# 0xWOLAND/halo2-prover

Hardware: AMD Instinct MI355X
Metric: MSM+NTT field-ops/s (higher is better)
Workload: dtype u32 limbs (256-bit modular)

## Files before the change

### halo2_prover_amd/csrc/h2_curve29.hpp

```cpp
#pragma once
#include "h2_curve.hpp"
#include "h2_field29.hpp"

namespace h2 {

constexpr int XYZZ29_WORDS = 36;

template <class CV>
struct Affine29 {
  using F = Fe29<typename CV::Base>;
  F x, y;
  H2_HD bool is_identity() const { return x.is_zero_exact() && y.is_zero_exact(); }
};

template <class CV>
struct Xyzz29 {
  using F = Fe29<typename CV::Base>;
  F x, y, zz, zzz;
  H2_HD bool is_identity() const { return zz.is_zero_exact(); }
  static H2_HD Xyzz29 identity() { return Xyzz29{F::zero(), F::zero(), F::zero(), F::zero()}; }
};

template <class CV>
H2_HD Affine29<CV> affine29_load(const void* p, bool negate) {
  using B = typename CV::Base;
  const char* c = reinterpret_cast<const char*>(p);
  Affine29<CV> a{fe29_unpack(fe_load<B>(c)), fe29_unpack(fe_load<B>(c + 32))};
  if (negate) a.y = fe29_neg(a.y);
  return a;
}
template <class CV>
H2_HD void affine29_store_table(void* p, const Affine<CV>& a) {
  using B = typename CV::Base;
  char* c = reinterpret_cast<char*>(p);
  if (a.is_identity()) {
    fe_store<B>(c, Fe<B>::zero());
    fe_store<B>(c + 32, Fe<B>::zero());
    return;
  }
  fe_store<B>(c, fe29_pack(fe29_from_api(a.x)));
  fe_store<B>(c + 32, fe29_pack(fe29_from_api(a.y)));
}

template <class CV>
H2_HD Xyzz29<CV> xyzz29_load(const uint32_t* p) {
  Xyzz29<CV> r;
#pragma unroll
  for (int i = 0; i < 9; i++) {
    r.x.v[i] = (int32_t)p[i];
    r.y.v[i] = (int32_t)p[9 + i];
    r.zz.v[i] = (int32_t)p[18 + i];
    r.zzz.v[i] = (int32_t)p[27 + i];
  }
  return r;
}
template <class CV>
H2_HD void xyzz29_store(uint32_t* p, const Xyzz29<CV>& a) {
#pragma unroll
  for (int i = 0; i < 9; i++) {
    p[i] = (uint32_t)a.x.v[i];
    p[9 + i] = (uint32_t)a.y.v[i];
    p[18 + i] = (uint32_t)a.zz.v[i];
    p[27 + i] = (uint32_t)a.zzz.v[i];
  }
}

template <class CV>
H2_HD Fe29<typename CV::Base> fe29_one() {
  using B = typename CV::Base;
  return fe29_from_api(Fe<B>::one());
}

template <class CV>
H2_HD Xyzz29<CV> xyzz29_from_affine(const Affine29<CV>& a) {
  if (a.is_identity()) return Xyzz29<CV>::identity();
  const Fe29<typename CV::Base> one = fe29_one<CV>();
  return Xyzz29<CV>{a.x, fe29_norm(a.y), one, one};
}

template <class CV>
H2_HD Xyzz29<CV> xyzz29_double_affine(const Affine29<CV>& a) {
  using F = Fe29<typename CV::Base>;
  if (a.is_identity() || fe29_is_zero_mod_p(a.y)) return Xyzz29<CV>::identity();
  const F u = fe29_norm(fe29_add(a.y, a.y));
  const F v = fe29_sqr(u);
  const F w = fe29_mul(u, v);
  const F s = fe29_mul(a.x, v);
  const F xx = fe29_sqr(a.x);
  const F m = fe29_norm(fe29_add(fe29_add(xx, xx), xx));
  const F x3 = fe29_norm(fe29_sub(fe29_sub(fe29_sqr(m), s), s));
  const F y3 = fe29_mul_sub(m, fe29_sub(s, x3), w, a.y);
  return Xyzz29<CV>{x3, y3, v, w};
}

template <class CV>
H2_HD Xyzz29<CV> xyzz29_double(const Xyzz29<CV>& p) {
  using F = Fe29<typename CV::Base>;
  if (p.is_identity() || fe29_is_zero_mod_p(p.y)) return Xyzz29<CV>::identity();
  const F u = fe29_norm(fe29_add(p.y, p.y));
  const F v = fe29_sqr(u);
  const F w = fe29_mul(u, v);
  const F s = fe29_mul(p.x, v);
  const F xx = fe29_sqr(p.x);
  const F m = fe29_norm(fe29_add(fe29_add(xx, xx), xx));
  const F x3 = fe29_norm(fe29_sub(fe29_sub(fe29_sqr(m), s), s));
  const F y3 = fe29_mul_sub(m, fe29_sub(s, x3), w, p.y);
  return Xyzz29<CV>{x3, y3, fe29_mul(v, p.zz), fe29_mul(w, p.zzz)};
}

template <class CV>
H2_HD Xyzz29<CV> xyzz29_add_affine(const Xyzz29<CV>& acc, const Affine29<CV>& q) {
  using F = Fe29<typename CV::Base>;
  if (q.is_identity()) return acc;
  if (acc.is_identity()) return xyzz29_from_affine(q);
  const F u2 = fe29_mul(q.x, acc.zz);
  const F s2 = fe29_mul(q.y, acc.zzz);
  const F p = fe29_sub(u2, acc.x);
  const F r = fe29_sub(s2, acc.y);
  if (fe29_is_zero_mod_p(p)) {
    if (fe29_is_zero_mod_p(r)) return xyzz29_double_affine(q);
    return Xyzz29<CV>::identity();
  }
  const F pp = fe29_sqr(p);
  const F ppp = fe29_mul(p, pp);
  const F qq = fe29_mul(acc.x, pp);
  const F x3 = fe29_norm(fe29_sub(fe29_sub(fe29_sub(fe29_sqr(r), ppp), qq), qq));
  const F y3 = fe29_mul_sub(r, fe29_sub(qq, x3), acc.y, ppp);
  return Xyzz29<CV>{x3, y3, fe29_mul(acc.zz, pp), fe29_mul(acc.zzz, ppp)};
}

template <class CV>
H2_HD Xyzz29<CV> xyzz29_add(const Xyzz29<CV>& a, const Xyzz29<CV>& b) {
  using F = Fe29<typename CV::Base>;
  if (a.is_identity()) return b;
  if (b.is_identity()) return a;
  const F u1 = fe29_mul(a.x, b.zz);
  const F u2 = fe29_mul(b.x, a.zz);
  const F s1 = fe29_mul(a.y, b.zzz);
  const F s2 = fe29_mul(b.y, a.zzz);
  const F p = fe29_sub(u2, u1);
  const F r = fe29_sub(s2, s1);
  if (fe29_is_zero_mod_p(p)) {
    if (fe29_is_zero_mod_p(r)) return xyzz29_double(a);
    return Xyzz29<CV>::identity();
  }
  const F pp = fe29_sqr(p);
  const F ppp = fe29_mul(p, pp);
  const F qq = fe29_mul(u1, pp);
  const F x3 = fe29_norm(fe29_sub(fe29_sub(fe29_sub(fe29_sqr(r), ppp), qq), qq));
  const F y3 = fe29_mul_sub(r, fe29_sub(qq, x3), s1, ppp);
  return Xyzz29<CV>{x3, y3, fe29_mul(fe29_mul(a.zz, b.zz), pp), fe29_mul(fe29_mul(a.zzz, b.zzz), ppp)};
}

template <class CV>
H2_HD Xyzz<CV> xyzz29_to_api(const Xyzz29<CV>& p) {
  if (p.is_identity()) return Xyzz<CV>::identity();
  return Xyzz<CV>{fe29_to_api(p.x), fe29_to_api(p.y), fe29_to_api(p.zz), fe29_to_api(p.zzz)};
}

}
```

### halo2_prover_amd/csrc/h2_field29.hpp

```cpp
#pragma once
#include "h2_field.hpp"

namespace h2 {

constexpr uint32_t L29_MASK = (1u << 29) - 1;

template <class FP>
struct Fe29 {
  int32_t v[9];
  static H2_HD Fe29 zero() {
    Fe29 r;
#pragma unroll
    for (int i = 0; i < 9; i++) r.v[i] = 0;
    return r;
  }
  H2_HD bool is_zero_exact() const {
    int32_t o = 0;
#pragma unroll
    for (int i = 0; i < 9; i++) o |= v[i];
    return o == 0;
  }
};

template <class FP>
H2_HD constexpr uint32_t fe29_p(int j) {
  const int bit = 29 * j;
  const int w = bit / 32, s = bit % 32;
  const uint64_t lo = w < 8 ? FP::P(w) : 0, hi = w + 1 < 8 ? FP::P(w + 1) : 0;
  return (uint32_t)(((lo | (hi << 32)) >> s) & L29_MASK);
}

template <class FP>
H2_HD Fe29<FP> fe29_unpack(const Fe<FP>& a) {
  Fe29<FP> r;
#pragma unroll
  for (int j = 0; j < 9; j++) {
    const int bit = 29 * j, w = bit >> 5, s = bit & 31;
    const uint64_t lo = a.v[w], hi = w + 1 < 8 ? a.v[w + 1] : 0;
    r.v[j] = (int32_t)((uint32_t)((lo | (hi << 32)) >> s) & L29_MASK);
  }
  return r;
}
template <class FP>
H2_HD Fe<FP> fe29_pack(const Fe29<FP>& a) {
  Fe<FP> r;
#pragma unroll
  for (int w = 0; w < 8; w++) {
    const int bit = 32 * w, j = bit / 29, off = bit % 29;
    uint64_t x = (uint64_t)(uint32_t)a.v[j] >> off;
    x |= (uint64_t)(uint32_t)a.v[j + 1] << (29 - off);
    if (j + 2 < 9) x |= (uint64_t)(uint32_t)a.v[j + 2] << (58 - off);
    r.v[w] = (uint32_t)x;
  }
  return r;
}

template <class FP>
H2_HD Fe29<FP> fe29_add(const Fe29<FP>& a, const Fe29<FP>& b) {
  Fe29<FP> r;
#pragma unroll
  for (int i = 0; i < 9; i++) r.v[i] = a.v[i] + b.v[i];
  return r;
}
template <class FP>
H2_HD Fe29<FP> fe29_sub(const Fe29<FP>& a, const Fe29<FP>& b) {
  Fe29<FP> r;
#pragma unroll
  for (int i = 0; i < 9; i++) r.v[i] = a.v[i] - b.v[i];
  return r;
}
template <class FP>
H2_HD Fe29<FP> fe29_neg(const Fe29<FP>& a) {
  Fe29<FP> r;
#pragma unroll
  for (int i = 0; i < 9; i++) r.v[i] = -a.v[i];
  return r;
}
template <class FP>
H2_HD Fe29<FP> fe29_norm(const Fe29<FP>& a) {
  Fe29<FP> r;
  int32_t carry = 0;
#pragma unroll
  for (int i = 0; i < 8; i++) {
    const int32_t x = a.v[i] + carry;
    r.v[i] = (int32_t)((uint32_t)x & L29_MASK);
    carry = x >> 29;
  }
  r.v[8] = a.v[8] + carry;
  return r;
}

H2_HD int32_t fe29_opaque(int32_t x) {
#if defined(__HIP_DEVICE_COMPILE__)
  asm("" : "+v"(x));
#endif
  return x;
}
namespace detail29 {
H2_HD int32_t fe29_hidden(int32_t c) {
#if defined(__HIP_DEVICE_COMPILE__)
  asm("" : "+s"(c));
#endif
  return c;
}
template <class FP, int J, bool UP>
H2_HD void msub_p(int64_t& acc, int32_t m) {
  constexpr uint32_t pj = fe29_p<FP>(J);
  if constexpr (UP) {
    if constexpr (pj == 0) {
    } else if constexpr (pj == 1) {
      acc += m;
    } else if constexpr ((pj & (pj - 1)) == 0) {
      acc += (int64_t)m << __builtin_ctz(pj);
    } else {
      acc += (int64_t)m * (int32_t)pj;
    }
  } else if constexpr (pj == 0) {
  } else if constexpr (__builtin_popcount(pj) <= 2) {
    acc += (int64_t)m * fe29_hidden(-(int32_t)pj);
  } else {
    acc += (int64_t)m * -(int32_t)pj;
  }
}
template <class FP, bool UP>
H2_HD int32_t mont_step(int64_t& acc) {
  constexpr uint32_t pinv = (0u - (FP::INV & L29_MASK)) & L29_MASK;
  if constexpr (UP) {
    constexpr uint32_t ninv = FP::INV & L29_MASK;
    const int32_t m = ninv == L29_MASK ? (int32_t)((0u - (uint32_t)acc) & L29_MASK)
                                       : (int32_t)(((uint32_t)acc * ninv) & L29_MASK);
    msub_p<FP, 0, true>(acc, m);
    return m;
  } else if constexpr (pinv == 1) {
    return fe29_opaque((int32_t)((uint32_t)acc & L29_MASK));
  } else {
    const int32_t m = fe29_opaque((int32_t)(((uint32_t)acc * pinv) & L29_MASK));
    msub_p<FP, 0, false>(acc, m);
    return m;
  }
}
template <class FP, int K, int I, int IEND>
H2_HD void col_ab(int64_t& acc, const int32_t* a, const int32_t* b) {
  if constexpr (I <= IEND) {
    acc += (int64_t)a[I] * b[K - I];
    col_ab<FP, K, I + 1, IEND>(acc, a, b);
  }
}
template <class FP, int K, int I, int IEND, bool UP>
H2_HD void col_mp(int64_t& acc, const int32_t* m) {
  if constexpr (I <= IEND) {
    msub_p<FP, K - I, UP>(acc, m[I]);
    col_mp<FP, K, I + 1, IEND, UP>(acc, m);
  }
}
template <class FP, int K, bool UP = false>
H2_HD void reduce_col(int64_t& acc, int32_t* m, int32_t* t) {
  if constexpr (K < 9) {
    if constexpr (K > 0) col_mp<FP, K, 0, K - 1, UP>(acc, m);
    m[K] = mont_step<FP, UP>(acc);
  } else {
    col_mp<FP, K, K - 8, 8, UP>(acc, m);
    t[K - 9] = (int32_t)((uint32_t)acc & L29_MASK);
  }
  acc >>= 29;
}
template <class FP, int K, bool UP = false>
H2_HD void columns(int64_t& acc, const int32_t* a, const int32_t* b, int32_t* m, int32_t* t) {
  if constexpr (K < 17) {
    col_ab<FP, K, (K < 9 ? 0 : K - 8), (K < 9 ? K : 8)>(acc, a, b);
    reduce_col<FP, K, UP>(acc, m, t);
    columns<FP, K + 1, UP>(acc, a, b, m, t);
  }
}
template <class FP, int K, int I, int IEND>
H2_HD void col_sq(int64_t& acc, const int32_t* a, const int32_t* a2) {
  if constexpr (I <= IEND) {
    if constexpr (I < K - I) acc += (int64_t)a[I] * a2[K - I];
    else if constexpr (I == K - I) acc += (int64_t)a[I] * a[I];
    col_sq<FP, K, I + 1, IEND>(acc, a, a2);
  }
}
template <class FP, int K>
H2_HD void columns_sq(int64_t& acc, const int32_t* a, const int32_t* a2, int32_t* m, int32_t* t) {
  if constexpr (K < 17) {
    col_sq<FP, K, (K < 9 ? 0 : K - 8), K / 2>(acc, a, a2);
    reduce_col<FP, K>(acc, m, t);
    columns_sq<FP, K + 1>(acc, a, a2, m, t);
  }
}
template <class FP, int K>
H2_HD void columns2(int64_t& acc, const int32_t* a, const int32_t* b, const int32_t* c, const int32_t* d, int32_t* m, int32_t* t) {
  if constexpr (K < 17) {
    col_ab<FP, K, (K < 9 ? 0 : K - 8), (K < 9 ? K : 8)>(acc, a, b);
    col_ab<FP, K, (K < 9 ? 0 : K - 8), (K < 9 ? K : 8)>(acc, c, d);
    reduce_col<FP, K>(acc, m, t);
    columns2<FP, K + 1>(acc, a, b, c, d, m, t);
  }
}
}

template <class FP>
H2_HD void fe29_opaque_limbs(int32_t* o, const Fe29<FP>& a) {
#pragma unroll
  for (int i = 0; i < 9; i++) o[i] = fe29_opaque(a.v[i]);
}

template <class FP>
H2_HD Fe29<FP> fe29_mul(const Fe29<FP>& a, const Fe29<FP>& b) {
  int64_t acc = 0;
  int32_t m[9], av[9], bv[9];
  fe29_opaque_limbs(av, a);
  fe29_opaque_limbs(bv, b);
  Fe29<FP> r;
  detail29::columns<FP, 0>(acc, av, bv, m, r.v);
  r.v[8] = (int32_t)acc;
  return r;
}
template <class FP>
H2_HD Fe29<FP> fe29_mul_plain(const Fe29<FP>& a, const Fe29<FP>& b) {
  int64_t acc = 0;
  int32_t m[9];
  Fe29<FP> r;
  detail29::columns<FP, 0>(acc, a.v, b.v, m, r.v);
  r.v[8] = (int32_t)acc;
  return r;
}
template <class FP>
H2_HD Fe29<FP> fe29_mul_up(const Fe29<FP>& a, const Fe29<FP>& b) {
  int64_t acc = 0;
  int32_t m[9], av[9], bv[9];
  fe29_opaque_limbs(av, a);
  fe29_opaque_limbs(bv, b);
  Fe29<FP> r;
  detail29::columns<FP, 0, true>(acc, av, bv, m, r.v);
  r.v[8] = (int32_t)acc;
  return r;
}
template <class FP>
H2_HD Fe29<FP> fe29_sqr(const Fe29<FP>& a) {
  int64_t acc = 0;
  int32_t m[9], av[9], a2[9];
  fe29_opaque_limbs(av, a);
#pragma unroll
  for (int i = 0; i < 9; i++) a2[i] = fe29_opaque(av[i] * 2);
  Fe29<FP> r;
  detail29::columns_sq<FP, 0>(acc, av, a2, m, r.v);
  r.v[8] = (int32_t)acc;
  return r;
}
template <class FP>
H2_HD Fe29<FP> fe29_mul_sub(const Fe29<FP>& a, const Fe29<FP>& b, const Fe29<FP>& c, const Fe29<FP>& d) {
  int64_t acc = 0;
  int32_t m[9], av[9], bv[9], nc[9], dv[9];
  fe29_opaque_limbs(av, a);
  fe29_opaque_limbs(bv, b);
  fe29_opaque_limbs(dv, d);
#pragma unroll
  for (int i = 0; i < 9; i++) nc[i] = fe29_opaque(-c.v[i]);
  Fe29<FP> r;
  detail29::columns2<FP, 0>(acc, av, bv, nc, dv, m, r.v);
  r.v[8] = (int32_t)acc;
  return r;
}

template <class FP>
H2_HD Fe29<FP> fe29_from_api(const Fe<FP>& a) {
  Fe<FP> t = a;
#pragma unroll
  for (int i = 0; i < 5; i++) t = fe_dbl(t);
  return fe29_unpack(t);
}
template <class FP>
H2_HD Fe<FP> fe29_canonical_pack(Fe29<FP> t) {
  Fe29<FP> pl;
#pragma unroll
  for (int i = 0; i < 9; i++) pl.v[i] = (int32_t)fe29_p<FP>(i);
  if (t.v[8] < 0) t = fe29_norm(fe29_add(t, pl));
  if (t.v[8] < 0) t = fe29_norm(fe29_add(t, pl));
  return fe29_pack(t);
}
template <class FP>
H2_HD Fe<FP> fe29_to_api(const Fe29<FP>& a) {
  Fe<FP> one;
#pragma unroll
  for (int i = 0; i < 8; i++) one.v[i] = FP::ONE(i);
  return fe29_canonical_pack(fe29_mul(a, fe29_unpack(one)));
}
template <class FP>
H2_HD Fe<FP> w_canonical_pack(const Fe29<FP>& t0) {
  Fe29<FP> pl;
#pragma unroll
  for (int i = 0; i < 9; i++) pl.v[i] = (int32_t)fe29_p<FP>(i);
  Fe29<FP> t = fe29_norm(t0);
  if (t.v[8] < 0) t = fe29_norm(fe29_add(t, pl));
  if (t.v[8] < 0) t = fe29_norm(fe29_add(t, pl));
  const Fe29<FP> s = fe29_norm(fe29_sub(t, pl));
  if (s.v[8] >= 0) t = s;
  return fe29_pack(t);
}

template <class FP>
H2_HD Fe29<FP> expr_column_operand(const Fe<FP>& a) {
  Fe29<FP> r;
#pragma unroll
  for (int j = 0; j < 9; j++) {
    const int bit = 29 * j - 5;
    uint32_t limb;
    if (bit < 0) {
      limb = (a.v[0] << 5) & L29_MASK;
    } else {
      const int w = bit >> 5, sh = bit & 31;
      const uint64_t lo = a.v[w], hi = w + 1 < 8 ? a.v[w + 1] : 0;
      limb = (uint32_t)((lo | (hi << 32)) >> sh) & L29_MASK;
    }
    const int pb = 29 * j - 4;
    uint32_t pl;
    if (pb < 0) {
      pl = (FP::P(0) << 4) & L29_MASK;
    } else {
      const int w = pb >> 5, sh = pb & 31;
      const uint64_t lo = w < 8 ? FP::P(w) : 0, hi = w + 1 < 8 ? FP::P(w + 1) : 0;
      pl = (uint32_t)((lo | (hi << 32)) >> sh) & L29_MASK;
    }
    r.v[j] = (int32_t)limb - (int32_t)pl;
  }
  return r;
}

template <class FP>
H2_HD Fe29<FP> fe29_inv(const Fe29<FP>& a) {
  const Fe29<FP> a2 = fe29_mul(a, a), a3 = fe29_mul(a2, a);
  uint32_t e[8];
  uint32_t borrow = 2;
#pragma unroll
  for (int i = 0; i < 8; i++) {
    const uint32_t w = FP::P(i);
    e[i] = w - borrow;
    borrow = w < borrow ? 1u : 0u;
  }
  Fe29<FP> r = fe29_from_api(Fe<FP>::one());
  for (int i = 254; i >= 0; i -= 2) {
    r = fe29_mul(r, r);
    r = fe29_mul(r, r);
    const uint32_t d = (e[i >> 5] >> (i & 31)) & 3u;
    if (d == 1) r = fe29_mul(r, a);
    else if (d == 2) r = fe29_mul(r, a2);
    else if (d == 3) r = fe29_mul(r, a3);
  }
  return r;
}

template <class FP>
H2_HD bool fe29_is_zero_mod_p(const Fe29<FP>& a) {
  constexpr uint32_t pinv = (0u - (FP::INV & L29_MASK)) & L29_MASK;
  const uint32_t j = ((uint32_t)a.v[0] * pinv) & L29_MASK;
  if (j > 16u && j < (1u << 29) - 16u) return false;
  return fe29_to_api(a).is_zero();
}

}
```

### halo2_prover_amd/csrc/h2_msm.hpp

```cpp
#pragma once
#include "h2_curve29.hpp"
#include "h2_curve_quad.hpp"
#include "h2_tune.hpp"
#include <hip/hip_ext.h>
#include <algorithm>
#include <cstdlib>

namespace h2 {

#ifdef H2_TAIL_STAMPS
__device__ unsigned long long* h2_stamps;
#define H2_STAMP(slot)                                                                                              \
  do {                                                                                                              \
    if (threadIdx.x == 0) h2_stamps[((size_t)blockIdx.y * gridDim.x + blockIdx.x) * 16 + (slot)] = wall_clock64(); \
  } while (0)
#else
#define H2_STAMP(slot)
#endif

constexpr uint32_t MSM_SIGN = 0x80000000u;
constexpr uint32_t MSM_MAX_WINDOWS = 48;
constexpr uint32_t MSM_HOT_SPAN = 256;
constexpr uint32_t MSM_HOT_SEG = 128;
constexpr uint32_t MSM_NOT_HOT = 0xFFFFFFFFu;
// ... 417 lines not shown
                   uint32_t tile, uint32_t tiles, uint32_t m, MsmGeom g) {
  using S = typename CV::Scalar;
  extern __shared__ uint32_t hist[];
  const MsmTileId id = msm_tile_id(tiles, m);
  if (!id.live) return;
  const uint32_t col = id.col;
  const uint32_t* tb = tile_base + ((size_t)col * tiles + id.tile) * g.B;
  const uint32_t* gc = gcounts + (size_t)col * g.B;
  const size_t K = (size_t)m * g.B;
  for (uint32_t b = threadIdx.x; b < g.B; b += blockDim.x) {
    uint32_t at = offsets[(size_t)col * g.B + b] + tb[b];
    for (uint32_t x = 0; x < id.group; x++) at += gc[x * K + b];
    hist[b] = at;
  }
  __syncthreads();
  const uint32_t lo = id.tile * tile, hi = min(lo + tile, n);
  for (uint32_t i = lo + threadIdx.x; i < hi; i += blockDim.x) {
    MsmDigits dg(fe_from_mont(fe_load<S>(scalars + 2 * (col_stride * col + i))).v);
    for (uint32_t w = 0; w < g.W; w++) {
      const uint32_t enc = dg.next(g, w);
      if (enc) {
        const uint32_t pos = atomicAdd(&hist[(enc & ~MSM_SIGN) - 1], 1u);
        sorted_ref[pos] = (w * n_bases + i) | (enc & MSM_SIGN);
      }
    }
  }
}

constexpr size_t MSM_STAGE_LDS_CAP = 160 * 1024 - 512;
struct MsmStagePack {
  uint32_t on;
  uint32_t bbits, ibits, wbits;
};
inline uint32_t msm_bits_for(uint64_t count) {
  uint32_t b = 0;
  while (((uint64_t)1 << b) < count) b++;
  return b;
}
inline MsmStagePack msm_stage_pack(const MsmGeom& g, size_t tile) {
  MsmStagePack p{};
  p.bbits = msm_bits_for(g.B);
  p.ibits = msm_bits_for(tile);
  p.wbits = msm_bits_for(g.W);
  p.on = p.bbits + p.ibits + p.wbits <= 31 ? 1u : 0u;
  return p;
}
inline size_t msm_stage_need(const MsmGeom& g, size_t tile, bool packed) {
  return (size_t)8 * g.B + (size_t)(packed ? 4 : 6) * tile * g.W + 64;
}
template <class CV, bool PACKED>
__global__ void __launch_bounds__(1024)
msm_scatter_staged_kernel(const U128* __restrict__ scalars, const uint32_t* __restrict__ offsets,
                          const uint32_t* __restrict__ gcounts, const uint32_t* __restrict__ tile_base,
                          const uint32_t* __restrict__ tile_hist, uint32_t* __restrict__ sorted_ref, uint32_t n,
                          size_t col_stride , uint32_t n_bases, uint32_t tile, uint32_t tiles, uint32_t m,
                          MsmGeom g, uint32_t stage_cap , MsmStagePack pk,
                          MsmKeysArgs keys) {
  using S = typename CV::Scalar;
  extern __shared__ uint32_t hist[];
  __shared__ uint32_t wave_sum[16];
  __shared__ uint32_t total_s;
  uint32_t* cur = hist;
  uint32_t* delta = hist + g.B;
  uint32_t* sref = hist + 2 * (size_t)g.B;
  uint16_t* sbkt = reinterpret_cast<uint16_t*>(sref + stage_cap);
  const MsmTileId id = msm_tile_id(tiles, m);
  if (!id.live) return;
  const uint32_t col = id.col;
  if (keys.keys_per_block) {
    const uint32_t v = col * tiles + id.tile;
    msm_keys_block(offsets, (size_t)m * g.B, keys, (size_t)v * keys.keys_per_block, keys.keys_per_block, v == 0, hist);
    __syncthreads();
  }
  const uint32_t* tb = tile_base + ((size_t)col * tiles + id.tile) * g.B;
  const uint32_t* th = tile_hist + ((size_t)col * tiles + id.tile) * g.B;
  const uint32_t* gc = gcounts + (size_t)col * g.B;
  const size_t K = (size_t)m * g.B;
  const uint32_t per = (g.B + blockDim.x - 1) / blockDim.x;
  const uint32_t b_lo = min(g.B, threadIdx.x * per), b_hi = min(g.B, b_lo + per);
  uint32_t s = 0;
  for (uint32_t b = b_lo; b < b_hi; b++) s += th[b];
  uint32_t incl = s;
  const uint32_t lane = threadIdx.x & 63, wave = threadIdx.x >> 6;
  for (uint32_t d = 1; d < 64; d <<= 1) {
    const uint32_t t = __shfl_up(incl, d, 64);
    if (lane >= d) incl += t;
  }
  if (lane == 63) wave_sum[wave] = incl;
  __syncthreads();
  uint32_t run = incl - s;
  for (uint32_t w = 0; w < wave; w++) run += wave_sum[w];
  for (uint32_t b = b_lo; b < b_hi; b++) {
    uint32_t at = offsets[(size_t)col * g.B + b] + tb[b];
    for (uint32_t x = 0; x < id.group; x++) at += gc[x * K + b];
    cur[b] = run;
    delta[b] = at - run;
    run += th[b];
  }
  if (threadIdx.x == blockDim.x - 1) total_s = run;
  __syncthreads();
  const uint32_t lo = id.tile * tile, hi = min(lo + tile, n);
  for (uint32_t i = lo + threadIdx.x; i < hi; i += blockDim.x) {
    MsmDigits dg(fe_from_mont(fe_load<S>(scalars + 2 * (col_stride * col + i))).v);
    for (uint32_t w = 0; w < g.W; w++) {
      const uint32_t enc = dg.next(g, w);
      if (enc) {
        const uint32_t b = (enc & ~MSM_SIGN) - 1;
        const uint32_t pos = atomicAdd(&cur[b], 1u);
        if (pos < stage_cap) {
          if (PACKED) {
            sref[pos] = b | ((i - lo) << pk.bbits) | (w << (pk.bbits + pk.ibits)) | (enc & MSM_SIGN);
          } else {
            sref[pos] = (w * n_bases + i) | (enc & MSM_SIGN);
            sbkt[pos] = (uint16_t)b;
          }
        }
      }
    }
  }
  __syncthreads();
  const uint32_t total = min(total_s, stage_cap);
  if (PACKED) {
    const uint32_t bmask = (1u << pk.bbits) - 1, imask = (1u << pk.ibits) - 1;
    for (uint32_t j = threadIdx.x; j < total; j += blockDim.x) {
      const uint32_t e = sref[j];
      const uint32_t w = (e & ~MSM_SIGN) >> (pk.bbits + pk.ibits), i = lo + ((e >> pk.bbits) & imask);
      sorted_ref[delta[e & bmask] + j] = (w * n_bases + i) | (e & MSM_SIGN);
    }
  } else {
    for (uint32_t j = threadIdx.x; j < total; j += blockDim.x) sorted_ref[delta[sbkt[j]] + j] = sref[j];
  }
}

template <class CV>
__device__ __forceinline__ Affine29<CV> msm_fetch(const U128* __restrict__ table, uint32_t entry) {
  return affine29_load<CV>(table + 4 * (size_t)(entry & ~MSM_SIGN), (entry & MSM_SIGN) != 0);
}

template <class CV>
__global__ void __launch_bounds__(256, MSM_CHUNK_WAVES)
msm_chunk_kernel(const U128* __restrict__ table, const U128* const* __restrict__ col_tables, uint32_t log_b,
                 const uint32_t* __restrict__ sorted_ref,
                 const uint32_t* __restrict__ chunk_first, const uint32_t* __restrict__ offsets, size_t K, uint32_t T_host,
                 uint32_t* __restrict__ bucket_sum, uint32_t* __restrict__ head, uint32_t* __restrict__ tail) {
  const uint32_t t = blockIdx.x * blockDim.x + threadIdx.x;
  const uint32_t E = offsets[K];
  const uint32_t T = msm_effective_t(E, T_host);
  const uint64_t lo64 = (uint64_t)t * T;
  if (lo64 >= E) return;
  const uint32_t lo = (uint32_t)lo64, hi = (uint32_t)min((uint64_t)E, lo64 + T);
  uint32_t key = chunk_first[t];
  uint32_t next = offsets[key + 1];
  if (col_tables) table = col_tables[key >> log_b];
  bool first = true;
  Xyzz29<CV> a = Xyzz29<CV>::identity();
  U128 quad = U128{0, 0, 0, 0};
  for (uint32_t e = lo; e < hi; e++) {
    if (e == lo || (e & 3u) == 0) quad = *reinterpret_cast<const U128*>(sorted_ref + (e & ~3u));
    const uint32_t sel = e & 3u;
    const uint32_t ref = sel == 0 ? quad.x : sel == 1 ? quad.y : sel == 2 ? quad.z : quad.w;
    if (e >= next) {
      if (first && offsets[key] != lo) xyzz29_store<CV>(head + XYZZ29_WORDS * (size_t)t, a);
      else xyzz29_store<CV>(bucket_sum + XYZZ29_WORDS * (size_t)key, a);
      first = false;
      a = Xyzz29<CV>::identity();
      do {
        key++;
        next = offsets[key + 1];
      } while (e >= next);
      if (col_tables) table = col_tables[key >> log_b];
    }
    a = xyzz29_add_affine(a, msm_fetch<CV>(table, ref));
  }
  const bool ends_here = next == hi;
  const bool starts_here = !first || offsets[key] == lo;
  if (starts_here && ends_here) xyzz29_store<CV>(bucket_sum + XYZZ29_WORDS * (size_t)key, a);
  else if (first) xyzz29_store<CV>(head + XYZZ29_WORDS * (size_t)t, a);
  else xyzz29_store<CV>(tail + XYZZ29_WORDS * (size_t)t, a);
}

template <class CV>
__device__ __forceinline__ Xyzz29<CV> xyzz_shfl_down(const Xyzz29<CV>& p, uint32_t delta) {
  Xyzz29<CV> r;
#pragma unroll
  for (int i = 0; i < 9; i++) {
    r.x.v[i] = __shfl_down(p.x.v[i], delta, 64);
    r.y.v[i] = __shfl_down(p.y.v[i], delta, 64);
    r.zz.v[i] = __shfl_down(p.zz.v[i], delta, 64);
    r.zzz.v[i] = __shfl_down(p.zzz.v[i], delta, 64);
  }
  return r;
}

__device__ __forceinline__ void h2_publish_release() {
  asm volatile("s_waitcnt vmcnt(0)" ::: "memory");
  __builtin_amdgcn_fence(__ATOMIC_RELEASE, "agent");
  asm volatile("s_waitcnt vmcnt(0)" ::: "memory");
}
__device__ __forceinline__ void h2_consume_acquire() {
  __builtin_amdgcn_fence(__ATOMIC_ACQUIRE, "agent");
  asm volatile("s_waitcnt vmcnt(0)" ::: "memory");
}

template <class CV>
__device__ __forceinline__ Xyzz29<CV> xyzz_fold_down(const Xyzz29<CV>& a, uint32_t d, uint32_t lane) {
  const Xyzz29<CV> o = xyzz_shfl_down(a, d);
  return lane < d ? xyzz29_add_quad(a, o) : a;
}

template <class CV>
__device__ __forceinline__ Xyzz29<CV> msm_piece(const uint32_t* __restrict__ head, const uint32_t* __restrict__ tail,
                                               uint32_t s, uint32_t j0, uint32_t T, uint32_t p) {
  const uint32_t j = j0 + p;
  const uint32_t* src = (p == 0 && s != j0 * T) ? tail : head;
  return xyzz29_load<CV>(src + XYZZ29_WORDS * (size_t)j);
}

inline uint32_t msm_fixup_task_blocks(uint32_t max_tasks) { return std::min<uint32_t>(256u, (max_tasks + 3) / 4); }
template <class CV>
__global__ void __launch_bounds__(256)
msm_fixup_kernel(const uint32_t* __restrict__ offsets, size_t K, uint32_t T_host, uint32_t log_g,
                 const uint32_t* __restrict__ bucket_sum, const uint32_t* __restrict__ head,
                 const uint32_t* __restrict__ tail, const uint32_t* __restrict__ hot_slot,
                 const uint32_t* __restrict__ tasks, const uint32_t* __restrict__ task_count, uint32_t max_tasks,
                 uint32_t task_blocks, uint32_t* hot_part, uint32_t* hot_arrive, uint32_t* __restrict__ xsum) {
  __builtin_amdgcn_s_setprio(3);
  const uint32_t T = msm_effective_t(offsets[K], T_host);
  if (blockIdx.x < task_blocks) {
    const uint32_t ntask = min(*task_count, max_tasks);
    const uint32_t lane = threadIdx.x & 63u, quad = lane >> 2;
    for (uint32_t t = blockIdx.x * 4 + (threadIdx.x >> 6); t < ntask; t += task_blocks * 4) {
      const uint32_t key = tasks[2 * t], q = tasks[2 * t + 1];
      const uint32_t s = offsets[key], e = offsets[key + 1];
      const uint32_t j0 = s / T, span = (e - 1) / T - j0 + 1;
      const uint32_t lo = q * MSM_HOT_SEG, hi = min(span, lo + MSM_HOT_SEG);
      const uint32_t nseg = (span + MSM_HOT_SEG - 1) / MSM_HOT_SEG, slot = hot_slot[key];
      uint32_t* part = hot_part + XYZZ29_WORDS * (size_t)slot;
      Xyzz29<CV> a = Xyzz29<CV>::identity();
      for (uint32_t p = lo + quad; p < hi; p += 16) a = xyzz29_add_quad(a, msm_piece<CV>(head, tail, s, j0, T, p));
      for (uint32_t d = 32; d >= 4; d >>= 1) a = xyzz_fold_down(a, d, lane);
      uint32_t arrived = 0;
      if (lane == 0) {
        xyzz29_store<CV>(part + XYZZ29_WORDS * (size_t)q, a);
        h2_publish_release();
        arrived = atomicAdd(hot_arrive + slot, 1u);
      }
      arrived = __shfl(arrived, 0, 64);
      if (arrived != nseg - 1) continue;
      h2_consume_acquire();
      a = Xyzz29<CV>::identity();
      for (uint32_t r = quad; r < nseg; r += 16) a = xyzz29_add_quad(a, xyzz29_load<CV>(part + XYZZ29_WORDS * (size_t)r));
      for (uint32_t d = 32; d >= 4; d >>= 1) a = xyzz_fold_down(a, d, lane);
      if (lane == 0) xyzz29_store<CV>(xsum + XYZZ29_WORDS * (size_t)key, a);
    }
    return;
  }
  const uint32_t G = 1u << log_g;
  const size_t gt = (size_t)(blockIdx.x - task_blocks) * blockDim.x + threadIdx.x;
  const size_t key = gt >> log_g;
  const uint32_t lane = (uint32_t)gt & (G - 1);
  const uint32_t quad = lane >> 2, nquad = G >> 2;
  bool live = key < K;
  Xyzz29<CV> x = Xyzz29<CV>::identity();
  if (live) {
    const uint32_t s = offsets[key], e = offsets[key + 1];
    if (e > s) {
      const uint32_t j0 = s / T, j1 = (e - 1) / T;
      if (j0 == j1) {
        if (quad == 0) x = xyzz29_load<CV>(bucket_sum + XYZZ29_WORDS * key);
      } else if (hot_slot[key] != MSM_NOT_HOT) {
        live = false;
      } else if (quad <= j1 - j0) {
        Xyzz29<CV> nxt = msm_piece<CV>(head, tail, s, j0, T, quad);
        for (uint32_t p = quad; p <= j1 - j0; p += nquad) {
          const Xyzz29<CV> cur = nxt;
          if (p + nquad <= j1 - j0) nxt = msm_piece<CV>(head, tail, s, j0, T, p + nquad);
          x = xyzz29_add_quad(x, cur);
        }
      }
    }
  }
  for (uint32_t d = G >> 1; d >= 4; d >>= 1) x = xyzz_fold_down(x, d, lane);
  if (live && lane == 0) xyzz29_store<CV>(xsum + XYZZ29_WORDS * key, x);
}

H2_HD bool msm_special_predoubled(uint32_t log_b, uint32_t lb) {
  const uint32_t hb = log_b - lb, ndig = ((hb + 1) >> 1) ? ((hb + 1) >> 1) : 1u;
  return lb >= 2 * ndig;
}
template <class CV>
__global__ void __launch_bounds__(256)
msm_rowcol_kernel(const uint32_t* __restrict__ xsum, uint32_t* __restrict__ rc, uint32_t* __restrict__ done,
                  uint32_t log_b, uint32_t lb, U128* zero_ptr = nullptr, uint32_t zero_u128 = 0) {
  __builtin_amdgcn_s_setprio(3);
  __shared__ uint32_t xw[3][XYZZ29_WORDS];
  const uint32_t col = blockIdx.y;
  if (blockIdx.x == 0 && threadIdx.x == 0) done[col] = 0;
  if (zero_ptr) {
    const uint32_t nthr = gridDim.x * gridDim.y * blockDim.x;
    for (uint32_t i = (blockIdx.y * gridDim.x + blockIdx.x) * blockDim.x + threadIdx.x; i < zero_u128; i += nthr)
      zero_ptr[i] = U128{0, 0, 0, 0};
  }
  const uint32_t rows = 1u << (log_b - lb), cols = 1u << lb;
  const bool is_row = blockIdx.x < rows;
  const uint32_t first = is_row ? blockIdx.x * cols : blockIdx.x - rows;
  const uint32_t stride = is_row ? 1u : cols, len = is_row ? cols : rows;
  const uint32_t* base = xsum + XYZZ29_WORDS * ((size_t)col << log_b);
  const uint32_t quad = threadIdx.x >> 2, nq = blockDim.x >> 2, lane = threadIdx.x & 63u, wave = threadIdx.x >> 6;
  Xyzz29<CV> a = quad < len ? xyzz29_load<CV>(base + XYZZ29_WORDS * (size_t)(first + quad * stride)) : Xyzz29<CV>::identity();
  if (quad + nq < len) {
    Xyzz29<CV> nxt = xyzz29_load<CV>(base + XYZZ29_WORDS * (size_t)(first + (quad + nq) * stride));
    for (uint32_t j = quad + nq; j < len; j += nq) {
      const Xyzz29<CV> cur = nxt;
      if (j + nq < len) nxt = xyzz29_load<CV>(base + XYZZ29_WORDS * (size_t)(first + (j + nq) * stride));
      a = xyzz29_add_quad(a, cur);
    }
  }
  for (uint32_t d = 32; d >= 4; d >>= 1) a = xyzz_fold_down(a, d, lane);
  if (blockDim.x > 64) {
    if (wave > 0 && lane == 0) xyzz29_store<CV>(xw[wave - 1], a);
    __syncthreads();
    if (wave > 0) return;
    const uint32_t nw = blockDim.x >> 6;
    if (quad >= 1) a = quad < nw ? xyzz29_load<CV>(xw[quad - 1]) : Xyzz29<CV>::identity();
    for (uint32_t d = 2 * nw; d >= 4; d >>= 1) a = xyzz_fold_down(a, d, lane);
// ... 699 lines not shown
```

### halo2_prover_amd/csrc/h2_selftest.hip

```cpp
#include "h2_internal.hpp"

#include <cstdio>

#include "../../include/h2hip_selftest.h"

using namespace h2;

extern "C" int h2_selftest_field_op(int field, int op, const uint64_t a[4], const uint64_t b[4], uint64_t out[4]) {
  if (!a || !b || !out) return H2_EINVAL;
  int rc = -1;
  switch (field) {
    case 0: rc = curve_ops_bn254()->selftest_field(0, op, a, b, out); break;
    case 1: rc = curve_ops_bn254()->selftest_field(1, op, a, b, out); break;
    case 2: rc = curve_ops_pallas()->selftest_field(0, op, a, b, out); break;
    case 3: rc = curve_ops_pallas()->selftest_field(1, op, a, b, out); break;
  }
  return rc == 0 ? H2_OK : H2_EINVAL;
}
template <class FP>
H2_HD void selftest_fe29_run(int op, const int32_t* in, int32_t* out) {
  Fe29<FP> a[4];
  for (int k = 0; k < 4; k++)
    for (int l = 0; l < 9; l++) a[k].v[l] = in[9 * k + l];
  Fe29<FP> r;
  switch (op) {
    case 0: r = fe29_mul(a[0], a[1]); break;
    case 1: r = fe29_sqr(a[0]); break;
    case 2: r = fe29_mul_sub(a[0], a[1], a[2], a[3]); break;
    default: r = fe29_mul_up(a[0], a[1]); break;
  }
  for (int l = 0; l < 9; l++) out[l] = r.v[l];
}
template <class FP>
__global__ void __launch_bounds__(64) selftest_fe29_kernel(int op, const int32_t* __restrict__ in, int32_t* __restrict__ out,
                                                           uint32_t n) {
  const uint32_t i = blockIdx.x * blockDim.x + threadIdx.x;
  if (i >= n) return;
  selftest_fe29_run<FP>(op, in + 36 * (size_t)i, out + 9 * (size_t)i);
}
extern "C" int h2_selftest_fe29_op(int field, int op, const int32_t in[36], int32_t out[9]) {
  if (!in || !out || op < 0 || op > 3) return H2_EINVAL;
  switch (field) {
    case 0: selftest_fe29_run<BN254_FQ>(op, in, out); return H2_OK;
    case 1: selftest_fe29_run<BN254_FR>(op, in, out); return H2_OK;
    case 2: selftest_fe29_run<PASTA_FP>(op, in, out); return H2_OK;
    case 3: selftest_fe29_run<PASTA_FQ>(op, in, out); return H2_OK;
  }
  return H2_EINVAL;
}
extern "C" int h2_selftest_fe29_op_device(int field, int op, const int32_t* in, int32_t* out, size_t n) {
  std::lock_guard<std::recursive_mutex> lk(g_h2_mu);
  if (!g_h2.ready) return H2_ENOTINIT;
  if (!in || !out || n == 0 || n > (1u << 20) || field < 0 || field > 3 || op < 0 || op > 3) return H2_EINVAL;
  DevCtx& g_ctx = g_h2.ctx[0];
  DeviceGuard dg(g_ctx.device);
  const size_t in_bytes = n * 36 * 4, out_bytes = n * 9 * 4;
  ArenaLease stage(g_ctx.stage, in_bytes + out_bytes, g_ctx.stream);
  if (stage.rc != H2_OK) return stage.rc;
  int32_t* d_in = (int32_t*)g_ctx.stage.p;
  int32_t* d_out = (int32_t*)((char*)g_ctx.stage.p + in_bytes);
  H2_TRY(hipMemcpyAsync(d_in, in, in_bytes, hipMemcpyHostToDevice, g_ctx.stream));
  const dim3 grid((unsigned)((n + 63) / 64)), block(64);
  switch (field) {
    case 0: hipLaunchKernelGGL(selftest_fe29_kernel<BN254_FQ>, grid, block, 0, g_ctx.stream, op, d_in, d_out, (uint32_t)n); break;
    case 1: hipLaunchKernelGGL(selftest_fe29_kernel<BN254_FR>, grid, block, 0, g_ctx.stream, op, d_in, d_out, (uint32_t)n); break;
    case 2: hipLaunchKernelGGL(selftest_fe29_kernel<PASTA_FP>, grid, block, 0, g_ctx.stream, op, d_in, d_out, (uint32_t)n); break;
    default: hipLaunchKernelGGL(selftest_fe29_kernel<PASTA_FQ>, grid, block, 0, g_ctx.stream, op, d_in, d_out, (uint32_t)n); break;
  }
  if (int rc = launched(hipGetLastError(), "selftest_fe29_kernel"); rc != H2_OK) return rc;
  H2_TRY(hipMemcpyAsync(out, d_out, out_bytes, hipMemcpyDeviceToHost, g_ctx.stream));
  return stage.wait();
}
extern "C" int h2_selftest_curve_op(int curve, int op, const uint64_t p[8], const uint64_t q[8], uint64_t out[8]) {
  const CurveOps* ops = ops_of(curve);
  if (!ops || !p || !q || !out) return H2_EINVAL;
  return ops->selftest_curve(op, p, q, out) == 0 ? H2_OK : H2_EINVAL;
}
extern "C" int h2_selftest_digits(int curve, const uint64_t scalar[4], size_t n_for_geometry, uint32_t* out,
                                  uint32_t cap) {
  const CurveOps* ops = ops_of(curve);
  if (!ops || !scalar || !out) return H2_EINVAL;
  return ops->selftest_digits(scalar, n_for_geometry, out, cap);
}
extern "C" int h2_selftest_curve_op_device(int curve, int op, const uint64_t* p, const uint64_t* q, uint64_t* out,
                                           size_t n) {
  std::lock_guard<std::recursive_mutex> lk(g_h2_mu);
  if (!g_h2.ready) return H2_ENOTINIT;
  const CurveOps* ops = ops_of(curve);
  if (!ops || !p || !q || !out || n == 0 || n > (1u << 20)) return H2_EINVAL;
  DevCtx& g_ctx = g_h2.ctx[0];
  DeviceGuard dg(g_ctx.device);
  ArenaLease stage(g_ctx.stage, 3 * n * 64, g_ctx.stream);
  if (stage.rc != H2_OK) return stage.rc;
  char* d = (char*)g_ctx.stage.p;
  H2_TRY(hipMemcpyAsync(d, p, n * 64, hipMemcpyHostToDevice, g_ctx.stream));
  H2_TRY(hipMemcpyAsync(d + n * 64, q, n * 64, hipMemcpyHostToDevice, g_ctx.stream));
  if (int rc = launched(ops->selftest_curve_device(op, d, d + n * 64, d + 2 * n * 64, (uint32_t)n, g_ctx.stream), "selftest_curve_kernel");
      rc != H2_OK)
    return rc;
  H2_TRY(hipMemcpyAsync(out, d + 2 * n * 64, n * 64, hipMemcpyDeviceToHost, g_ctx.stream));
  return stage.wait();
}

extern "C" int h2_selftest_field_op_device(int field, int op, const uint64_t* a, const uint64_t* b, uint64_t* out,
                                           size_t n) {
  std::lock_guard<std::recursive_mutex> lk(g_h2_mu);
  if (!g_h2.ready) return H2_ENOTINIT;
  if (!a || !b || !out || n == 0 || n > (1u << 24) || field < 0 || field > 3) return H2_EINVAL;
  const CurveOps* ops = field < 2 ? curve_ops_bn254() : curve_ops_pallas();
  const int which = field & 1;
  DevCtx& g_ctx = g_h2.ctx[0];
  DeviceGuard dg(g_ctx.device);
  ArenaLease stage(g_ctx.stage, 3 * n * 32, g_ctx.stream);
  if (stage.rc != H2_OK) return stage.rc;
  char* d = (char*)g_ctx.stage.p;
  H2_TRY(hipMemcpyAsync(d, a, n * 32, hipMemcpyHostToDevice, g_ctx.stream));
  H2_TRY(hipMemcpyAsync(d + n * 32, b, n * 32, hipMemcpyHostToDevice, g_ctx.stream));
  if (int rc = launched(ops->selftest_field_device(which, op, d, d + n * 32, d + 2 * n * 32, (uint32_t)n, g_ctx.stream), "selftest_field_kernel");
      rc != H2_OK)
    return rc;
  H2_TRY(hipMemcpyAsync(out, d + 2 * n * 32, n * 32, hipMemcpyDeviceToHost, g_ctx.stream));
  return stage.wait();
}

extern "C" int h2_selftest_msm_guard(int on) {
  std::lock_guard<std::recursive_mutex> lk(g_h2_mu);
  g_knobs.msm_guard = on != 0;
  g_knobs.msm_guard_poke = on == 2;
  g_knobs.sort2_pack = on != 3;
  g_counts.guard_launches = g_counts.guard_violations = 0;
  g_counts.guard_first.clear();
  return H2_OK;
}
extern "C" int h2_selftest_msm_guard_report(uint64_t out[2], char* first, size_t cap) {
  std::lock_guard<std::recursive_mutex> lk(g_h2_mu);
  if (!out) return H2_EINVAL;
  out[0] = g_counts.guard_launches;
  out[1] = g_counts.guard_violations;
  if (first && cap) {
    snprintf(first, cap, "%s", g_counts.guard_first.c_str());
  }
  return H2_OK;
}
extern "C" int h2_selftest_msm_check(int curve, size_t n_bases, size_t n, size_t m, size_t col_stride, int guard, uint64_t out[8]) {
  std::lock_guard<std::recursive_mutex> lk(g_h2_mu);
  const CurveOps* ops = ops_of(curve);
  if (!ops || n == 0 || m == 0 || n > n_bases) return H2_EINVAL;
  const MsmGeom g = msm_geometry(n_bases, ops->scalar_bits);
  const MsmGroupPlan plan = msm_plan_group(g, n_bases, n, m, col_stride, guard != 0, true);
  if (plan.cols == 0) return H2_EINVAL;
  if (m > plan.cols && col_stride < n) { g_h2.last_error = "msm launch geometry: col_stride >= n"; return H2_EINVAL; }
  const MsmWorkspace& ws = plan.ws;
  if (out) {
    out[0] = g.c; out[1] = g.W; out[2] = g.B; out[3] = ws.sort2 ? ws.s2.tile : ws.tile;
    out[4] = ws.staged; out[5] = ws.sort2; out[6] = ws.T; out[7] = ws.n_regions;
  }
  if (plan.broken) {
    g_h2.last_error = std::string("msm launch geometry: ") + plan.broken;
    return H2_EINVAL;
  }
  return H2_OK;
}
extern "C" int h2_selftest_msm_points_check(int curve, size_t n, size_t m, size_t col_stride, int guard, uint64_t out[8]) {
  std::lock_guard<std::recursive_mutex> lk(g_h2_mu);
  if (!curve_ok(curve) || !out || n == 0 || m == 0 || n > MSM_POINTS_MAX_N) return H2_EINVAL;
  if (col_stride < n) { g_h2.last_error = "msm points launch geometry: col_stride >= n"; return H2_EINVAL; }
  const MsmGeom g = msm_points_geometry(n, ops_of(curve)->scalar_bits);
  const MsmGroupPlan plan = msm_points_plan_group(g, n, m, col_stride, guard != 0);
  if (plan.cols == 0) return H2_EINVAL;
  const MsmWorkspace& ws = plan.ws;
  out[0] = g.c; out[1] = g.W; out[2] = g.B; out[3] = ws.tile; out[4] = (uint64_t)g.W * g.B * 4; out[5] = plan.cols;
  out[6] = ws.T; out[7] = ws.n_regions;
  if (plan.broken) {
    g_h2.last_error = std::string("msm points launch geometry: ") + plan.broken;
    return H2_EDEVICE;
  }
  return H2_OK;
}
extern "C" int h2_selftest_set_msm_points_small_max(size_t n) {
  std::lock_guard<std::recursive_mutex> lk(g_h2_mu);
  g_knobs.points_small_max = n == SIZE_MAX ? MSM_POINTS_SMALL_MAX : n;
  return H2_OK;
}
extern "C" int h2_selftest_msm_front(int curve, size_t n_bases, size_t n, size_t m, int pack, uint64_t out[12]) {
  std::lock_guard<std::recursive_mutex> lk(g_h2_mu);
  const CurveOps* ops = ops_of(curve);
  if (!ops || !out || n == 0 || m == 0 || n > n_bases || n_bases >= (1ull << 31)) return H2_EINVAL;
  const MsmGeom g = msm_geometry(n_bases, ops->scalar_bits);
  const MsmGroupPlan plan = msm_plan_group(g, n_bases, n, m, n, false, pack != 0);
  if (plan.cols < m) return H2_EINVAL;
  const MsmWorkspace& ws = plan.ws;
  const char* broken = plan.broken;
  if (broken) g_h2.last_error = std::string("msm launch geometry: ") + broken;
  out[0] = ws.sort2 ? ws.s2.tile : ws.tile; out[1] = ws.staged; out[2] = ws.stage_lds; out[3] = ws.pack.on;
  out[4] = ws.pack.bbits; out[5] = ws.pack.ibits; out[6] = ws.pack.wbits; out[7] = broken ? 0 : 1;
  out[8] = msm_effective_t((uint32_t)ws.E, ws.T); out[9] = MSM_HOT_SPAN; out[10] = MSM_HOT_SEG; out[11] = ws.max_tasks;
  return H2_OK;
}
extern "C" int h2_selftest_arena_stats(uint64_t out[4]) {
  std::lock_guard<std::recursive_mutex> lk(g_h2_mu);
  DevCtx* c = g_h2.ready ? ctx_current() : nullptr;
  if (!c || !out) return H2_EINVAL;
  out[0] = g_counts.arena_growths;
  out[1] = g_counts.arena_waits;
  out[2] = c->msm_ws.takeovers;
  out[3] = c->ntt_ws.takeovers;
// ... 35 lines not shown
```

Before: 186.9 billion.

## Make MSM bucket accumulation branch-light and add single-chain pinned Montgomery variants

The bucket accumulation loop in the 29-bit MSM kernel now starts each bucket by loading the first point directly. Later additions go through a new in-place affine add that always runs the general formula and only branches into a slow path that re-fetches the point for the rare identity or doubling cases. This reduces divergence and register pressure from carrying the point across the branch, at the cost of recomputing a fetch in those edge cases. It also adds an opt-in Chain::One variant of the field mul/sqr kernels, which pins the 64-bit accumulator with empty asm to force a single serial chain. That variant is only exercised by new selftest ops, so it is not used by default.

```diff
diff --git a/halo2_prover_amd/csrc/h2_curve29.hpp b/halo2_prover_amd/csrc/h2_curve29.hpp
--- a/halo2_prover_amd/csrc/h2_curve29.hpp
+++ b/halo2_prover_amd/csrc/h2_curve29.hpp
@@ -129,6 +129,30 @@
   return Xyzz29<CV>{x3, y3, fe29_mul(acc.zz, pp), fe29_mul(acc.zzz, ppp)};
 }
 
+template <class CV, class Refetch>
+H2_HD void xyzz29_acc_affine(Xyzz29<CV>& acc, const Affine29<CV>& q, Refetch refetch) {
+  using F = Fe29<typename CV::Base>;
+  if (q.is_identity()) return;
+  const bool acc_id = acc.is_identity();
+  const F u2 = fe29_mul(q.x, acc.zz);
+  const F s2 = fe29_mul(q.y, acc.zzz);
+  const F p = fe29_sub(u2, acc.x);
+  const F r = fe29_sub(s2, acc.y);
+  const bool pz = !acc_id && fe29_is_zero_mod_p(p);
+  const bool dbl = pz && fe29_is_zero_mod_p(r);
+  const F pp = fe29_sqr(p);
+  const F ppp = fe29_mul(p, pp);
+  const F qq = fe29_mul(acc.x, pp);
+  acc.x = fe29_norm(fe29_sub(fe29_sub(fe29_sub(fe29_sqr(r), ppp), qq), qq));
+  acc.y = fe29_mul_sub(r, fe29_sub(qq, acc.x), acc.y, ppp);
+  acc.zz = fe29_mul(acc.zz, pp);
+  acc.zzz = fe29_mul(acc.zzz, ppp);
+  if (acc_id || pz) {
+    const Affine29<CV> q2 = refetch();
+    acc = acc_id ? xyzz29_from_affine(q2) : dbl ? xyzz29_double_affine(q2) : Xyzz29<CV>::identity();
+  }
+}
+
 template <class CV>
 H2_HD Xyzz29<CV> xyzz29_add(const Xyzz29<CV>& a, const Xyzz29<CV>& b) {
   using F = Fe29<typename CV::Base>;
diff --git a/halo2_prover_amd/csrc/h2_field29.hpp b/halo2_prover_amd/csrc/h2_field29.hpp
--- a/halo2_prover_amd/csrc/h2_field29.hpp
+++ b/halo2_prover_amd/csrc/h2_field29.hpp
@@ -4,6 +4,8 @@
 namespace h2 {
 
 constexpr uint32_t L29_MASK = (1u << 29) - 1;
+
+enum class Chain { Two, One };
 
 template <class FP>
 struct Fe29 {
@@ -139,62 +141,72 @@
     return m;
   }
 }
-template <class FP, int K, int I, int IEND>
+template <bool PIN>
+H2_HD void pin(int64_t& acc) {
+#if defined(__HIP_DEVICE_COMPILE__)
+  if constexpr (PIN) asm("" : "+v"(acc));
+#endif
+}
+template <class FP, int K, int I, int IEND, bool PIN = false>
 H2_HD void col_ab(int64_t& acc, const int32_t* a, const int32_t* b) {
   if constexpr (I <= IEND) {
     acc += (int64_t)a[I] * b[K - I];
-    col_ab<FP, K, I + 1, IEND>(acc, a, b);
-  }
-}
-template <class FP, int K, int I, int IEND, bool UP>
+    pin<PIN>(acc);
+    col_ab<FP, K, I + 1, IEND, PIN>(acc, a, b);
+  }
+}
+template <class FP, int K, int I, int IEND, bool UP, bool PIN = false>
 H2_HD void col_mp(int64_t& acc, const int32_t* m) {
   if constexpr (I <= IEND) {
     msub_p<FP, K - I, UP>(acc, m[I]);
-    col_mp<FP, K, I + 1, IEND, UP>(acc, m);
-  }
-}
-template <class FP, int K, bool UP = false>
+    if constexpr (fe29_p<FP>(K - I) != 0) pin<PIN>(acc);
+    col_mp<FP, K, I + 1, IEND, UP, PIN>(acc, m);
+  }
+}
+template <class FP, int K, bool UP = false, bool PIN = false>
 H2_HD void reduce_col(int64_t& acc, int32_t* m, int32_t* t) {
   if constexpr (K < 9) {
-    if constexpr (K > 0) col_mp<FP, K, 0, K - 1, UP>(acc, m);
+    if constexpr (K > 0) col_mp<FP, K, 0, K - 1, UP, PIN>(acc, m);
     m[K] = mont_step<FP, UP>(acc);
   } else {
-    col_mp<FP, K, K - 8, 8, UP>(acc, m);
+    col_mp<FP, K, K - 8, 8, UP, PIN>(acc, m);
     t[K - 9] = (int32_t)((uint32_t)acc & L29_MASK);
   }
   acc >>= 29;
-}
-template <class FP, int K, bool UP = false>
+  if constexpr (K < 16) pin<PIN>(acc);
+}
+template <class FP, int K, bool UP = false, Chain CH = Chain::Two>
 H2_HD void columns(int64_t& acc, const int32_t* a, const int32_t* b, int32_t* m, int32_t* t) {
   if constexpr (K < 17) {
-    col_ab<FP, K, (K < 9 ? 0 : K - 8), (K < 9 ? K : 8)>(acc, a, b);
-    reduce_col<FP, K, UP>(acc, m, t);
-    columns<FP, K + 1, UP>(acc, a, b, m, t);
-  }
-}
-template <class FP, int K, int I, int IEND>
+    col_ab<FP, K, (K < 9 ? 0 : K - 8), (K < 9 ? K : 8), CH == Chain::One>(acc, a, b);
+    reduce_col<FP, K, UP, CH == Chain::One>(acc, m, t);
+    columns<FP, K + 1, UP, CH>(acc, a, b, m, t);
+  }
+}
+template <class FP, int K, int I, int IEND, bool PIN = false>
 H2_HD void col_sq(int64_t& acc, const int32_t* a, const int32_t* a2) {
   if constexpr (I <= IEND) {
     if constexpr (I < K - I) acc += (int64_t)a[I] * a2[K - I];
     else if constexpr (I == K - I) acc += (int64_t)a[I] * a[I];
-    col_sq<FP, K, I + 1, IEND>(acc, a, a2);
-  }
-}
-template <class FP, int K>
+    pin<PIN>(acc);
+    col_sq<FP, K, I + 1, IEND, PIN>(acc, a, a2);
+  }
+}
+template <class FP, int K, Chain CH = Chain::Two>
 H2_HD void columns_sq(int64_t& acc, const int32_t* a, const int32_t* a2, int32_t* m, int32_t* t) {
   if constexpr (K < 17) {
-    col_sq<FP, K, (K < 9 ? 0 : K - 8), K / 2>(acc, a, a2);
-    reduce_col<FP, K>(acc, m, t);
-    columns_sq<FP, K + 1>(acc, a, a2, m, t);
-  }
-}
-template <class FP, int K>
+    col_sq<FP, K, (K < 9 ? 0 : K - 8), K / 2, CH == Chain::One>(acc, a, a2);
+    reduce_col<FP, K, false, CH == Chain::One>(acc, m, t);
+    columns_sq<FP, K + 1, CH>(acc, a, a2, m, t);
+  }
+}
+template <class FP, int K, Chain CH = Chain::Two>
 H2_HD void columns2(int64_t& acc, const int32_t* a, const int32_t* b, const int32_t* c, const int32_t* d, int32_t* m, int32_t* t) {
   if constexpr (K < 17) {
-    col_ab<FP, K, (K < 9 ? 0 : K - 8), (K < 9 ? K : 8)>(acc, a, b);
-    col_ab<FP, K, (K < 9 ? 0 : K - 8), (K < 9 ? K : 8)>(acc, c, d);
-    reduce_col<FP, K>(acc, m, t);
-    columns2<FP, K + 1>(acc, a, b, c, d, m, t);
+    col_ab<FP, K, (K < 9 ? 0 : K - 8), (K < 9 ? K : 8), CH == Chain::One>(acc, a, b);
+    col_ab<FP, K, (K < 9 ? 0 : K - 8), (K < 9 ? K : 8), CH == Chain::One>(acc, c, d);
+    reduce_col<FP, K, false, CH == Chain::One>(acc, m, t);
+    columns2<FP, K + 1, CH>(acc, a, b, c, d, m, t);
   }
 }
 }
@@ -205,14 +217,14 @@
   for (int i = 0; i < 9; i++) o[i] = fe29_opaque(a.v[i]);
 }
 
-template <class FP>
+template <Chain CH = Chain::Two, class FP>
 H2_HD Fe29<FP> fe29_mul(const Fe29<FP>& a, const Fe29<FP>& b) {
   int64_t acc = 0;
   int32_t m[9], av[9], bv[9];
   fe29_opaque_limbs(av, a);
   fe29_opaque_limbs(bv, b);
   Fe29<FP> r;
-  detail29::columns<FP, 0>(acc, av, bv, m, r.v);
+  detail29::columns<FP, 0, false, CH>(acc, av, bv, m, r.v);
   r.v[8] = (int32_t)acc;
   return r;
 }
@@ -225,18 +237,18 @@
   r.v[8] = (int32_t)acc;
   return r;
 }
-template <class FP>
+template <Chain CH = Chain::Two, class FP>
 H2_HD Fe29<FP> fe29_mul_up(const Fe29<FP>& a, const Fe29<FP>& b) {
   int64_t acc = 0;
   int32_t m[9], av[9], bv[9];
   fe29_opaque_limbs(av, a);
   fe29_opaque_limbs(bv, b);
   Fe29<FP> r;
-  detail29::columns<FP, 0, true>(acc, av, bv, m, r.v);
-  r.v[8] = (int32_t)acc;
-  return r;
-}
-template <class FP>
+  detail29::columns<FP, 0, true, CH>(acc, av, bv, m, r.v);
+  r.v[8] = (int32_t)acc;
+  return r;
+}
+template <Chain CH = Chain::Two, class FP>
 H2_HD Fe29<FP> fe29_sqr(const Fe29<FP>& a) {
   int64_t acc = 0;
   int32_t m[9], av[9], a2[9];
@@ -244,11 +256,11 @@
 #pragma unroll
   for (int i = 0; i < 9; i++) a2[i] = fe29_opaque(av[i] * 2);
   Fe29<FP> r;
-  detail29::columns_sq<FP, 0>(acc, av, a2, m, r.v);
-  r.v[8] = (int32_t)acc;
-  return r;
-}
-template <class FP>
+  detail29::columns_sq<FP, 0, CH>(acc, av, a2, m, r.v);
+  r.v[8] = (int32_t)acc;
+  return r;
+}
+template <Chain CH = Chain::Two, class FP>
 H2_HD Fe29<FP> fe29_mul_sub(const Fe29<FP>& a, const Fe29<FP>& b, const Fe29<FP>& c, const Fe29<FP>& d) {
   int64_t acc = 0;
   int32_t m[9], av[9], bv[9], nc[9], dv[9];
@@ -258,7 +270,7 @@
 #pragma unroll
   for (int i = 0; i < 9; i++) nc[i] = fe29_opaque(-c.v[i]);
   Fe29<FP> r;
-  detail29::columns2<FP, 0>(acc, av, bv, nc, dv, m, r.v);
+  detail29::columns2<FP, 0, CH>(acc, av, bv, nc, dv, m, r.v);
   r.v[8] = (int32_t)acc;
   return r;
 }
diff --git a/halo2_prover_amd/csrc/h2_msm.hpp b/halo2_prover_amd/csrc/h2_msm.hpp
--- a/halo2_prover_amd/csrc/h2_msm.hpp
+++ b/halo2_prover_amd/csrc/h2_msm.hpp
@@ -593,7 +593,7 @@
   uint32_t key = chunk_first[t];
   uint32_t next = offsets[key + 1];
   if (col_tables) table = col_tables[key >> log_b];
-  bool first = true;
+  bool first = true, fresh = true;
   Xyzz29<CV> a = Xyzz29<CV>::identity();
   U128 quad = U128{0, 0, 0, 0};
   for (uint32_t e = lo; e < hi; e++) {
@@ -604,14 +604,20 @@
       if (first && offsets[key] != lo) xyzz29_store<CV>(head + XYZZ29_WORDS * (size_t)t, a);
       else xyzz29_store<CV>(bucket_sum + XYZZ29_WORDS * (size_t)key, a);
       first = false;
-      a = Xyzz29<CV>::identity();
+      fresh = true;
       do {
         key++;
         next = offsets[key + 1];
       } while (e >= next);
       if (col_tables) table = col_tables[key >> log_b];
     }
-    a = xyzz29_add_affine(a, msm_fetch<CV>(table, ref));
+    const Affine29<CV> q = msm_fetch<CV>(table, ref);
+    if (fresh) {
+      a = xyzz29_from_affine(q);
+      fresh = false;
+    } else {
+      xyzz29_acc_affine(a, q, [&] { return msm_fetch<CV>(table, ref); });
+    }
   }
   const bool ends_here = next == hi;
   const bool starts_here = !first || offsets[key] == lo;
diff --git a/halo2_prover_amd/csrc/h2_selftest.hip b/halo2_prover_amd/csrc/h2_selftest.hip
--- a/halo2_prover_amd/csrc/h2_selftest.hip
+++ b/halo2_prover_amd/csrc/h2_selftest.hip
@@ -27,7 +27,11 @@
     case 0: r = fe29_mul(a[0], a[1]); break;
     case 1: r = fe29_sqr(a[0]); break;
     case 2: r = fe29_mul_sub(a[0], a[1], a[2], a[3]); break;
-    default: r = fe29_mul_up(a[0], a[1]); break;
+    case 3: r = fe29_mul_up(a[0], a[1]); break;
+    case 4: r = fe29_mul<Chain::One>(a[0], a[1]); break;
+    case 5: r = fe29_sqr<Chain::One>(a[0]); break;
+    case 6: r = fe29_mul_sub<Chain::One>(a[0], a[1], a[2], a[3]); break;
+    default: r = fe29_mul_up<Chain::One>(a[0], a[1]); break;
   }
   for (int l = 0; l < 9; l++) out[l] = r.v[l];
 }
@@ -39,7 +43,7 @@
   selftest_fe29_run<FP>(op, in + 36 * (size_t)i, out + 9 * (size_t)i);
 }
 extern "C" int h2_selftest_fe29_op(int field, int op, const int32_t in[36], int32_t out[9]) {
-  if (!in || !out || op < 0 || op > 3) return H2_EINVAL;
+  if (!in || !out || op < 0 || op > 7) return H2_EINVAL;
   switch (field) {
     case 0: selftest_fe29_run<BN254_FQ>(op, in, out); return H2_OK;
     case 1: selftest_fe29_run<BN254_FR>(op, in, out); return H2_OK;
@@ -51,7 +55,7 @@
 extern "C" int h2_selftest_fe29_op_device(int field, int op, const int32_t* in, int32_t* out, size_t n) {
   std::lock_guard<std::recursive_mutex> lk(g_h2_mu);
   if (!g_h2.ready) return H2_ENOTINIT;
-  if (!in || !out || n == 0 || n > (1u << 20) || field < 0 || field > 3 || op < 0 || op > 3) return H2_EINVAL;
+  if (!in || !out || n == 0 || n > (1u << 20) || field < 0 || field > 3 || op < 0 || op > 7) return H2_EINVAL;
   DevCtx& g_ctx = g_h2.ctx[0];
   DeviceGuard dg(g_ctx.device);
   const size_t in_bytes = n * 36 * 4, out_bytes = n * 9 * 4;
```

Result: no change. 187.5 billion (median of 5 runs) (+0.3%).
